# efeslab/Atom

Hardware: AMD Instinct MI355X
Metric: effective TOPS, W4A4 group-128 GEMM + 128 INT8 outlier cols, fp16 out (higher is better)
Workload: dtype int4xint4 exact integer dot (BF6-coded on the f8f6f4 MFMA; INT8 MFMA for the keeper), fp32 dequant, fp16 out

## Files before the change

atom_amd/csrc/gemm_w4a4_f6.hip:

```cpp
#include <type_traits>
#include "common.h"
#include "quant_math.h"

namespace atom {

__global__ void splitk_reduce_kernel(const float *ws, half_t *D, int64_t MN, int splits);

namespace f6 {

typedef const __attribute__((address_space(1))) void *gptr_t;
typedef __attribute__((address_space(3))) void *lptr_t;
typedef int v8i __attribute__((ext_vector_type(8)));
typedef float v16f __attribute__((ext_vector_type(16)));

constexpr int TN = 2;
constexpr int PITCH = 104;
constexpr float kMagic = 12582912.0f;
constexpr int kMagicBits = 0x4B400000;

template <int BM_, int BN_, int TM_, int NS_, int OCC_ = 2, int FS_ = 0>
struct Cfg {
  static constexpr int FS = FS_;
  static constexpr int FS32 = FS_ == 1;
  static constexpr int OCC = OCC_;
// ... 1068 lines not shown
    auto dmak1 = [&](int i) { if (i == 0) issue_keeper<C>(p, 1, slot_of(G + 1), wave, lane, m0, n0); };
    auto tr_sel = [&]() {
      if constexpr ((ABL & 16) != 0) {
        if (tr_on) tr_i += 6;
        tr_on = blockIdx.x == 0 && tr_i + 6 <= 78 && (s < 3 || s == G / 2 || s == G / 2 + 1 || s + 3 >= G);
      }
    };
    kstamp(3);
    if constexpr ((ABL & 1024) != 0) {
      auto dma4f = [&](int i) { if (i < C::GLDS) issue_int4_piece<C>(p, s + 2, lds + 2 * C::STAGE_BYTES, wave, lane, m0, n0, i); };
      for (; s + 2 < G; ++s) p_step<C, false, ABL>(R, lds, lds + C::STAGE_BYTES, wm, wn, lane, c, sync, dma4f, stamp);
    }
    for (; s + 2 < G; ++s) { tr_sel(); p_step<C, false, ABL>(R, slot_of(s), slot_of(s + 1), wm, wn, lane, c, sync, dma4, stamp); }
    if (G >= 2) { tr_sel(); p_step<C, false, ABL>(R, slot_of(s), slot_of(s + 1), wm, wn, lane, c, sync, dmak0, stamp); ++s; }
    tr_sel();
    p_step<C, true, ABL>(R, slot_of(s), slot_of(s + 1), wm, wn, lane, c, sync, dmak1, stamp);
  }
  kstamp(4);
  p_drain<C>(R, c);
  kstamp(5);
  asm volatile("s_waitcnt vmcnt(0)" ::: "memory");
  __builtin_amdgcn_s_barrier();
  kstamp(6);
  if constexpr (!(ABL & 128)) p_keeper<C>(slot_of(G), slot_of(G + 1), wm, wn, lane, c);
  kstamp(7);

#pragma unroll
  for (int tb = 0; tb < 8; ++tb) {
    const int m = m0 + wm * 128 + p_row(tb) + 2 * l15;
    if (m >= p.M) continue;
#pragma unroll
    for (int h = 0; h < 2; ++h) {
      const int n = n0 + wn * 64 + 32 * h + 8 * kb;
      if (n >= p.N) continue;
      v4u o;
      half_t *ov = reinterpret_cast<half_t *>(&o);
#pragma unroll
      for (int r = 0; r < 4; ++r) {
        ov[2 * r] = f2h(c[2 * h][tb][r]);
        ov[2 * r + 1] = f2h(c[2 * h + 1][tb][r]);
      }
      if constexpr ((ABL & 64) != 0) { if (o.x != 0x12345678u) continue; }
      *reinterpret_cast<v4u *>(p.D + (int64_t)m * p.N + n) = o;
    }
  }
  if constexpr ((ABL & 16) != 0) {
    kstamp(8);
    asm volatile("s_waitcnt vmcnt(0)" ::: "memory");
    kstamp(9);
    if (blockIdx.x == 0) {
      if (lane == 0) trl[79] = (unsigned)__builtin_amdgcn_s_memrealtime();
      asm volatile("s_waitcnt lgkmcnt(0)" ::: "memory");
      for (int i = lane; i < 80; i += 64) reinterpret_cast<unsigned *>(p.Dsz)[wave * 80 + i] = trl[i];
    }
  }
}

template <class C>
struct QC {
  static constexpr int SB_OFF = C::SB_OFF;
  static constexpr int STAGE = C::SB_OFF + C::BN * 4;
  static constexpr int LDS_BYTES = 3 * STAGE;
  static_assert(LDS_BYTES <= 160 * 1024 && STAGE + (32 * 3 + 1) * PITCH + 100 < 65536, "q kernel: stage layout / ds offsets");
};

typedef float v2f_t __attribute__((ext_vector_type(2)));
#ifdef ATOM_SA_B32
struct QSa {
  float v;
  __device__ __forceinline__ QSa() = default;
  __device__ __forceinline__ QSa(float f) : v(f) {}
  __device__ __forceinline__ operator float() const { return v; }
};
#else
struct QSa {
  v2f_t p;
  __device__ __forceinline__ QSa() = default;
  __device__ __forceinline__ QSa(float f) : p{0.f, f} {}
  __device__ __forceinline__ QSa(v2f_t q) : p(q) {}
  __device__ __forceinline__ operator float() const { asm volatile("" ::"v"(p)); return p.y; }
};
#endif

template <class C, bool PAIR = false>
struct QRegs {
  v8i af[4];
  v8i bf[3];
  float sb[2][PAIR ? 4 : 8];
  QSa sa[4];
  v4f_t acc[2][2];
  int aW[2][3], aA[2][3], aS[2], aB[2];
#ifdef ATOM_F6_PAIR128
  int aWp[2][3];
#endif
};

template <int SL> __device__ __forceinline__ constexpr int q_set() { return SL == 2 ? 1 : 0; }
template <class C, int SL> __device__ __forceinline__ constexpr int q_imm() { return SL == 1 ? QC<C>::STAGE : 0; }

template <class C, int SL>
__device__ __forceinline__ v8i q_frag(const char *lds, const int (&a)[2][3], int off, int ro) {
  const char *b = lds + (SL < 0 ? ro : q_imm<C, SL>()) + off;
  const v2u x = *reinterpret_cast<const v2u *>(b + a[q_set<SL>()][0]);
  const v2u y = *reinterpret_cast<const v2u *>(b + a[q_set<SL>()][1]);
  const v2u z = *reinterpret_cast<const v2u *>(b + a[q_set<SL>()][2]);
  asm volatile("" ::: "memory");
  return v8i{(int)x.x, (int)x.y, (int)y.x, (int)y.y, (int)z.x, (int)z.y, 0, 0};
}
#ifdef ATOM_F6_PAIR128
template <class C, int SL>
__device__ __forceinline__ void q_frag_pair(const char *lds, const int (&a)[2][3], int off, int ro, v8i &f0, v8i &f1) {
  const char *b = lds + (SL < 0 ? ro : q_imm<C, SL>()) + off;
  const v4u x = *reinterpret_cast<const v4u *>(b + a[q_set<SL>()][0]);
  const v4u y = *reinterpret_cast<const v4u *>(b + a[q_set<SL>()][1]);
  const v4u z = *reinterpret_cast<const v4u *>(b + a[q_set<SL>()][2]);
  asm volatile("" ::: "memory");
  f0 = v8i{(int)x.x, (int)x.y, (int)y.x, (int)y.y, (int)z.x, (int)z.y, 0, 0};
  f1 = v8i{(int)x.z, (int)x.w, (int)y.z, (int)y.w, (int)z.z, (int)z.w, 0, 0};
}
#endif
template <class C, int SL, class RG>
__device__ __forceinline__ QSa q_scale(const char *lds, const RG &R, int off, int ro) {
#ifdef ATOM_SA_B32
  return *reinterpret_cast<const float *>(lds + (SL < 0 ? ro : q_imm<C, SL>()) + off + R.aS[q_set<SL>()] + 4);
#else
  return QSa(*reinterpret_cast<const v2f_t *>(lds + (SL < 0 ? ro : q_imm<C, SL>()) + off + R.aS[q_set<SL>()]));
#endif
}
template <class C, int SL, class RG>
__device__ __forceinline__ void q_load_sb(const char *lds, RG &R, int h, int ro) {
  const char *b = lds + (SL < 0 ? ro : q_imm<C, SL>()) + QC<C>::SB_OFF + 128 * h + R.aB[q_set<SL>()];
  if constexpr (sizeof(R.sb[0]) == 4 * sizeof(float)) {
    const float *f = reinterpret_cast<const float *>(b);
#pragma unroll
    for (int k = 0; k < 4; ++k) R.sb[h][k] = f[2 * k];
  } else {
    const v4f_t lo = *reinterpret_cast<const v4f_t *>(b), hi = *reinterpret_cast<const v4f_t *>(b + 16);
#pragma unroll
    for (int k = 0; k < 4; ++k) { R.sb[h][k] = lo[k]; R.sb[h][4 + k] = hi[k]; }
  }
}

__device__ __forceinline__ void q_dma16x3(unsigned m0v, unsigned voff, const void *sbase) {
  asm volatile("s_mov_b32 m0, %0\n\ts_nop 0\n\tglobal_load_lds_dwordx4 %1, %2\n\tglobal_load_lds_dwordx4 %1, %2 offset:1024\n\t"
               "global_load_lds_dwordx4 %1, %2 offset:2048" ::"s"(m0v), "v"(voff), "s"(sbase) : "memory");
}
__device__ __forceinline__ void q_dma16(unsigned m0v, unsigned voff, const void *sbase) {
  asm volatile("s_mov_b32 m0, %0\n\ts_nop 0\n\tglobal_load_lds_dwordx4 %1, %2" ::"s"(m0v), "v"(voff), "s"(sbase) : "memory");
}
struct QDma {
  unsigned voffW, voffA, voffX;
  int m0W, m0A, m0X;
  int xkind;
};
template <class C, int DS>
__device__ __forceinline__ void q_piece(const QDma &d, const uint8_t *wsrc, const uint8_t *asrc, const float *sbsrc, int i) {
  constexpr int base = DS * QC<C>::STAGE;
  if (i == 0) q_dma16x3(base + d.m0W, d.voffW, wsrc);
  else if (i == 3) q_dma16x3(base + d.m0A, d.voffA, asrc);
  else if (i == 6) {
    const void *xb = d.xkind == 1 ? (const void *)wsrc : (d.xkind == 2 ? (const void *)asrc : (const void *)sbsrc);
    q_dma16(base + d.m0X, d.voffX, xb);
  }
}

struct QNoEarly { __device__ __forceinline__ void operator()(int) const {} };
template <class C, int SL, bool PAIR, class FS, class FD, class FE = QNoEarly>
__device__ __forceinline__ void q_step(QRegs<C, PAIR> &R, const char *lds, float (&c)[4][8][4], FS sync, FD mid, int ro = 0, int rn = 0,
                                       bool LAST = false, FE early = FE(), unsigned *tp = nullptr) {
  constexpr int NX = SL < 0 ? -1 : (SL + 1) % 3;
  auto stamp = [&](int k) {
    if (tp) { __builtin_amdgcn_sched_barrier(0); const unsigned t_ = (unsigned)__builtin_amdgcn_s_memtime(); if ((threadIdx.x & 63) == 0) tp[k] = t_; __builtin_amdgcn_sched_barrier(0); }
  };
#pragma unroll
  for (int i = 0; i < 16; ++i) {
    const int tb = p_tb(i), h = p_h(i);
    __builtin_amdgcn_sched_barrier(0);
    stamp(i);
    if (i == 8) { stamp(16); sync(); stamp(17); }
    __builtin_amdgcn_sched_barrier(0);
#pragma unroll
    for (int k = 0; k < 2; ++k)
      R.acc[i & 1][k] = __builtin_amdgcn_mfma_scale_f32_16x16x128_f8f6f4(R.af[2 * h + k], R.bf[p_buf(tb)], v4f_t{0.f, 0.f, 0.f, 0.f}, 3, 3, 0, 0, 0, 0);
    __builtin_amdgcn_sched_barrier(0);
    stamp(32 + 2 * i);
    if (h == 1 && i < 12 && tb + 2 < 8) {
      R.bf[p_buf(tb + 2)] = q_frag<C, SL>(lds, R.aA, p_row(tb + 2) * PITCH, ro);
      R.sa[(tb + 2) & 3] = q_scale<C, SL>(lds, R, p_row(tb + 2) * PITCH, ro);
    }
    if (!LAST) {
      if (i == 12) {
        R.bf[2] = q_frag<C, NX>(lds, R.aA, p_row(0) * PITCH, rn);
        R.sa[0] = q_scale<C, NX>(lds, R, p_row(0) * PITCH, rn);
      }
      if (i == 13) {
#ifdef ATOM_F6_PAIR128
        q_frag_pair<C, NX>(lds, R.aWp, p_row(0) * PITCH, rn, R.af[0], R.af[1]);
#else
        R.af[0] = q_frag<C, NX>(lds, R.aW, p_row(0) * PITCH, rn);
        R.af[1] = q_frag<C, NX>(lds, R.aW, p_row(1) * PITCH, rn);
#endif
      }
      if (i == 15) {
#ifdef ATOM_F6_PAIR128
        q_frag_pair<C, NX>(lds, R.aWp, p_row(2) * PITCH, rn, R.af[2], R.af[3]);
#else
        R.af[2] = q_frag<C, NX>(lds, R.aW, p_row(2) * PITCH, rn);
        R.af[3] = q_frag<C, NX>(lds, R.aW, p_row(3) * PITCH, rn);
#endif
        R.bf[1] = q_frag<C, NX>(lds, R.aA, p_row(1) * PITCH, rn);
        R.sa[1] = q_scale<C, NX>(lds, R, p_row(1) * PITCH, rn);
      }
    }
    if (i >= 8) mid(i - 8);
    else early(i);
    if (tp) asm volatile("s_waitcnt lgkmcnt(0)" ::: "memory");
    stamp(33 + 2 * i);
    __builtin_amdgcn_sched_barrier(0);
    {
      const int j = (i + 15) & 15, dtb = p_tb(j), dh = p_h(j);
      deq_pair<PAIR>(R.acc[j & 1][0], R.acc[j & 1][1], R.sa[dtb & 3], R.sb[dh], c[2 * dh][dtb], c[2 * dh + 1][dtb]);
    }
    __builtin_amdgcn_sched_barrier(0);
    if (!LAST && i == 14) q_load_sb<C, NX>(lds, R, 0, rn);
    if (i == 0) q_load_sb<C, SL>(lds, R, 1, ro);
  }
  stamp(18);
}

template <class C, bool STORE, int NTB>
__device__ __forceinline__ void q_keeper(const GemmParams &p, const char *slot, const char *slot1, int wm, int wn, int lane, float (&c)[4][NTB][4],
                                         int m0, int n0) {
  constexpr bool MERGED = true;
  const int l15 = lane & 15, kb = lane >> 4;
  const int sw = (l15 >> 1) & 3;
  const char *pw = slot + (wn * 64 + 2 * l15) * 64 + ((kb ^ sw) << 4);
  const char *pa = slot + (C::BN + wm * (16 * NTB) + 2 * l15) * 64 + ((kb ^ sw) << 4);
  const char *psa = slot + C::KP_SA_OFF + (wm * (16 * NTB) + 2 * l15) * 4;
  const char *psb = slot + C::SB_OFF + (wn * 64 + 8 * kb) * 2;
  v4i af[4], bf[2];
  v4i af1[4], bf1[2];
  const long d1 = slot1 - slot;
  float sb[2][8], sa[2];
  v4i acc[2][2];
  const v4i magic = {kMagicBits, kMagicBits, kMagicBits, kMagicBits};
#pragma unroll
  for (int fb = 0; fb < 4; ++fb) af[fb] = __builtin_bit_cast(v4i, *reinterpret_cast<const v4u *>(pw + p_row(fb) * 64));
  bf[0] = __builtin_bit_cast(v4i, *reinterpret_cast<const v4u *>(pa + p_row(0) * 64));
  bf[1] = __builtin_bit_cast(v4i, *reinterpret_cast<const v4u *>(pa + p_row(1) * 64));
  if constexpr (MERGED) {
#pragma unroll
    for (int fb = 0; fb < 4; ++fb) af1[fb] = __builtin_bit_cast(v4i, *reinterpret_cast<const v4u *>(pw + d1 + p_row(fb) * 64));
    bf1[0] = __builtin_bit_cast(v4i, *reinterpret_cast<const v4u *>(pa + d1 + p_row(0) * 64));
    bf1[1] = __builtin_bit_cast(v4i, *reinterpret_cast<const v4u *>(pa + d1 + p_row(1) * 64));
  }
  half_t sah[2];
  sah[0] = *reinterpret_cast<const half_t *>(psa + p_row(0) * 4);
  sah[1] = *reinterpret_cast<const half_t *>(psa + p_row(1) * 4);
#pragma unroll
  for (int h = 0; h < 2; ++h) {
    const v4u w = *reinterpret_cast<const v4u *>(psb + 64 * h);
    const half_t *hv = reinterpret_cast<const half_t *>(&w);
#pragma unroll
    for (int j = 0; j < 8; ++j) { sb[h][j] = (float)hv[j]; asm volatile("" : "+v"(sb[h][j])); }
  }
  auto store_block = [&](int tb) {
    const int m = m0 + wm * (16 * NTB) + p_row(tb) + 2 * l15;
    if (m >= p.M) return;
#pragma unroll
    for (int h = 0; h < 2; ++h) {
      const int n = n0 + wn * 64 + 32 * h + 8 * kb;
      if (n >= p.N) continue;
      v4u o;
      half_t *ov = reinterpret_cast<half_t *>(&o);
#pragma unroll
      for (int r = 0; r < 4; ++r) {
        ov[2 * r] = f2h(c[2 * h][tb][r]);
        ov[2 * r + 1] = f2h(c[2 * h + 1][tb][r]);
      }
      *reinterpret_cast<v4u *>(p.D + (int64_t)m * p.N + n) = o;
    }
  };
  auto dequant = [&](int j) {
    const int tb = j >> 1, h = j & 1;
    v4f_t f[2];
#pragma unroll
    for (int k = 0; k < 2; ++k)
#pragma unroll
      for (int r = 0; r < 4; ++r) f[k][r] = __int_as_float(acc[j & 1][k][r]) - kMagic;
    deq_pair<false>(f[0], f[1], sa[tb & 1], sb[h], c[2 * h][tb], c[2 * h + 1][tb]);
  };
#pragma unroll
  for (int i = 0; i < 2 * NTB; ++i) {
    const int tb = i >> 1, h = i & 1;
    __builtin_amdgcn_sched_barrier(0);
    if (h == 0) sa[tb & 1] = (float)sah[tb & 1];
#pragma unroll
    for (int k = 0; k < 2; ++k) acc[i & 1][k] = __builtin_amdgcn_mfma_i32_16x16x64_i8(af[2 * h + k], bf[tb & 1], magic, 0, 0, 0);
    if constexpr (MERGED) {
#pragma unroll
      for (int k = 0; k < 2; ++k) acc[i & 1][k] = __builtin_amdgcn_mfma_i32_16x16x64_i8(af1[2 * h + k], bf1[tb & 1], acc[i & 1][k], 0, 0, 0);
    }
    __builtin_amdgcn_sched_barrier(0);
    if (h == 1 && tb + 2 < NTB) {
      bf[tb & 1] = __builtin_bit_cast(v4i, *reinterpret_cast<const v4u *>(pa + p_row(tb + 2) * 64));
      if constexpr (MERGED) bf1[tb & 1] = __builtin_bit_cast(v4i, *reinterpret_cast<const v4u *>(pa + d1 + p_row(tb + 2) * 64));
      sah[tb & 1] = *reinterpret_cast<const half_t *>(psa + p_row(tb + 2) * 4);
    }
    if constexpr (STORE) { if (h == 1 && tb >= 1) store_block(tb - 1); }
    __builtin_amdgcn_sched_barrier(0);
    if (i > 0) dequant(i - 1);
  }
  __builtin_amdgcn_sched_barrier(0);
  dequant(2 * NTB - 1);
  if constexpr (STORE) store_block(NTB - 1);
}

template <class C, int GU = 0, bool TR = false, bool PAIR = false>
__global__ __launch_bounds__(C::NT, C::OCC) void gemm_w4a4_f6q_kernel(GemmParams p) {
  extern __shared__ __attribute__((aligned(16))) char lds[];
  static_assert(C::BM == 256 && C::BN == 256 && C::WM == 128 && C::NS == 3 && C::NW == 8, "q kernel: 256x256, 8 waves of 64 x 128");
  using Q = QC<C>;
  unsigned *trb = nullptr;
  auto kstamp = [&](int k) {
    if constexpr (TR) {
      if (trb) { const unsigned t = (unsigned)__builtin_amdgcn_s_memtime(); if ((threadIdx.x & 63) == 0) trb[k] = t; }
    }
  };
  if constexpr (TR) {
    if (blockIdx.x == 0 || blockIdx.x == gridDim.x - 1) {
      trb = reinterpret_cast<unsigned *>(p.Dsz) + ((blockIdx.x ? 8 : 0) + (threadIdx.x >> 6)) * 128;
      if ((threadIdx.x & 63) == 0) trb[62] = (unsigned)__builtin_amdgcn_s_memrealtime();
    }
    kstamp(0);
  }
  const int tid = threadIdx.x;
  const int lane = tid & 63;
  const int wave = __builtin_amdgcn_readfirstlane(tid >> 6);
  __builtin_assume(wave >= 0 && wave < C::NW);
  const int wm = wave / C::WGN, wn = wave % C::WGN;
  const int nbn = (p.N + C::BN - 1) / C::BN, nbm = (p.M + C::BM - 1) / C::BM;
  const int nwg = nbm * nbn;
  int id = blockIdx.x;
  {
    const int q = nwg >> 3, r = nwg & 7, xcd = id & 7, k = id >> 3;
    id = (xcd < r ? xcd * (q + 1) : r * (q + 1) + (xcd - r) * q) + k;
  }
  constexpr int GM = 4;
  const int band = id / (GM * nbn), inband = id % (GM * nbn);
  const int rows_in_band = min(GM, nbm - band * GM);
  const int bm = band * GM + inband % rows_in_band, bn = inband / rows_in_band;
  const int m0 = bm * C::BM, n0 = bn * C::BN;

  float c[4][8][4];
#pragma unroll
  for (int a = 0; a < 4; ++a)
#pragma unroll
    for (int b = 0; b < 8; ++b)
#pragma unroll
      for (int r = 0; r < 4; ++r) c[a][b][r] = 0.f;

  const int G = p.G;
  QDma d;
  d.voffW = d.voffA = (unsigned)(wave * 3072 + lane * 16);
  d.m0W = wave * 3072;
  d.m0A = C::A_OFF + wave * 3072;
  d.xkind = wave < 2 ? 1 : (wave < 4 ? 2 : 3);
  d.voffX = (unsigned)((wave < 4 ? (24 + (wave & 1)) * 1024 : 0) + lane * 16);
  d.m0X = wave < 2 ? (24 + wave) * 1024 : (wave < 4 ? C::A_OFF + (24 + (wave & 1)) * 1024 : Q::SB_OFF);
  const int64_t wstep = p.f6_rows_b * PITCH, astep = p.f6_rows_a * PITCH;
  const uint8_t *wsrc0 = p.B4 + (int64_t)n0 * PITCH, *asrc0 = p.A4 + (int64_t)m0 * PITCH;
  const float *sbsrc0 = p.sB32 + n0;
  auto slot_of = [&](int stage) { return lds + (stage % 3) * Q::STAGE; };
  auto issue_all = [&](auto ds, int g) {
    constexpr int DS = decltype(ds)::value;
#pragma unroll
    for (int i = 0; i < 7; ++i) q_piece<C, DS>(d, wsrc0 + g * wstep, asrc0 + g * astep, sbsrc0 + (int64_t)g * p.f6_rows_b, i);
  };
  const bool early1 = G >= 6;
  issue_all(std::integral_constant<int, 0>(), 0);
  if (!early1) {
    if (G >= 2) issue_all(std::integral_constant<int, 1>(), 1);
    else issue_keeper<C>(p, 0, slot_of(1), wave, lane, m0, n0);
  }
  kstamp(1);
  asm volatile("s_waitcnt vmcnt(0)" ::: "memory");
  __builtin_amdgcn_s_barrier();
  kstamp(2);

  const int l15 = lane & 15, kb = lane >> 4;
  QRegs<C, PAIR> R;
  {
    const int lw = wn * 64 * PITCH + l15 * (2 * PITCH) + kb * 24;
    const int la = C::A_OFF + wm * 128 * PITCH + l15 * (2 * PITCH);
#pragma unroll
    for (int st = 0; st < 2; ++st) {
#pragma unroll
      for (int k = 0; k < 3; ++k) {
        R.aW[st][k] = lw + 8 * k + st * 2 * Q::STAGE;
        R.aA[st][k] = la + kb * 24 + 8 * k + st * 2 * Q::STAGE;
        asm volatile("" : "+v"(R.aW[st][k]), "+v"(R.aA[st][k]));
#ifdef ATOM_F6_PAIR128
        R.aWp[st][k] = ((wn * 64 * PITCH + l15 * (2 * PITCH) + kb * 48 + 16 * k + st * 2 * Q::STAGE) & ~15);
        asm volatile("" : "+v"(R.aWp[st][k]));
#endif
      }
      R.aS[st] = la + 96 + st * 2 * Q::STAGE;
      R.aB[st] = (wn * 64 + 8 * kb) * 4 + st * 2 * Q::STAGE;
      asm volatile("" : "+v"(R.aS[st]), "+v"(R.aB[st]));
    }
    R.bf[2] = q_frag<C, 0>(lds, R.aA, p_row(0) * PITCH, 0);
#pragma unroll
    for (int fb = 0; fb < 4; ++fb) R.af[fb] = q_frag<C, 0>(lds, R.aW, p_row(fb) * PITCH, 0);
    R.bf[1] = q_frag<C, 0>(lds, R.aA, p_row(1) * PITCH, 0);
    R.bf[0] = R.bf[1];
    R.sa[0] = q_scale<C, 0>(lds, R, p_row(0) * PITCH, 0);
    R.sa[1] = q_scale<C, 0>(lds, R, p_row(1) * PITCH, 0);
    R.sa[2] = 0.f;
    R.sa[3] = 0.f;
    q_load_sb<C, 0>(lds, R, 0, 0);
    q_load_sb<C, 0>(lds, R, 1, 0);
#pragma unroll
    for (int k = 0; k < 2; ++k) R.acc[1][k] = v4f_t{0.f, 0.f, 0.f, 0.f};
  }
  if constexpr (TR) { asm volatile("s_waitcnt lgkmcnt(0)" ::: "memory"); kstamp(3); }
  auto sync = [&]() {
    asm volatile("s_waitcnt vmcnt(0)" ::: "memory");
    __builtin_amdgcn_s_barrier();
  };
  auto reg = [&](auto sl, int s) {
    constexpr int SL = decltype(sl)::value;
    if constexpr (TR) { if (s < 44) kstamp(16 + s); }
    const int g = s + 2;
    const uint8_t *wsrc = wsrc0 + g * wstep, *asrc = asrc0 + g * astep;
    const float *sbsrc = sbsrc0 + (int64_t)g * p.f6_rows_b;
    unsigned *tp = nullptr;
    if constexpr (TR) { if (trb && s == 9) tp = trb + 64; }
    q_step<C, SL, PAIR>(R, lds, c, sync, [&](int i) { q_piece<C, (SL + 2) % 3>(d, wsrc, asrc, sbsrc, i); }, 0, 0, false, QNoEarly(), tp);
  };
  using S0 = std::integral_constant<int, 0>;
  using S1 = std::integral_constant<int, 1>;
  using S2 = std::integral_constant<int, 2>;
  int s = 0;
  if (early1) {
    if constexpr (TR) kstamp(16);
    const uint8_t *wsrc = wsrc0 + 2 * wstep, *asrc = asrc0 + 2 * astep;
    const float *sbsrc = sbsrc0 + (int64_t)2 * p.f6_rows_b;
    q_step<C, 0, PAIR>(R, lds, c, sync, [&](int i) { q_piece<C, 2>(d, wsrc, asrc, sbsrc, i); }, 0, 0, false,
                 [&](int i) { q_piece<C, 1>(d, wsrc0 + wstep, asrc0 + astep, sbsrc0 + p.f6_rows_b, i); });
    reg(S1(), 1);
    reg(S2(), 2);
    s = 3;
  }
  for (; s + 4 < G; s += 3) { reg(S0(), s); reg(S1(), s + 1); reg(S2(), s + 2); }
  if (s + 2 < G) { reg(S0(), s); ++s; }
  if (s + 2 < G) { reg(S1(), s); ++s; }
  for (; s < G; ++s) {
    if constexpr (TR) { if (s < 44) kstamp(16 + s); }
    const int g = s + 2;
    const int dsl = g % 3;
    const uint8_t *wsrc = wsrc0 + g * wstep, *asrc = asrc0 + g * astep;
    const float *sbsrc = sbsrc0 + (int64_t)g * p.f6_rows_b;
    q_step<C, -1, PAIR>(R, lds, c, sync,
                  [&](int i) {
                    if (g < G) {
                      if (dsl == 0) q_piece<C, 0>(d, wsrc, asrc, sbsrc, i);
                      else if (dsl == 1) q_piece<C, 1>(d, wsrc, asrc, sbsrc, i);
                      else q_piece<C, 2>(d, wsrc, asrc, sbsrc, i);
                    } else if (i == 0) issue_keeper<C>(p, g - G, slot_of(g), wave, lane, m0, n0);
                  },
                  (s % 3) * Q::STAGE, ((s + 1) % 3) * Q::STAGE, s + 1 == G);
  }
  deq_pair<PAIR>(R.acc[1][0], R.acc[1][1], R.sa[3], R.sb[1], c[2][7], c[3][7]);
  kstamp(4);
  asm volatile("s_waitcnt vmcnt(0)" ::: "memory");
  __builtin_amdgcn_s_barrier();
  kstamp(5); kstamp(6);
  q_keeper<C, GU == 0>(p, slot_of(G), slot_of(G + 1), wm, wn, lane, c, m0, n0);
  if constexpr (TR) {
    kstamp(7);
    asm volatile("s_waitcnt vmcnt(0)" ::: "memory");
    kstamp(8);
    if (trb && (threadIdx.x & 63) == 0) trb[63] = (unsigned)__builtin_amdgcn_s_memrealtime();
  }
  if constexpr (GU == 0) return;

  if constexpr (GU != 0) {
    constexpr bool SIM = GU == 1;
    float *am = reinterpret_cast<float *>(lds + ((G + 2) % 3) * Q::STAGE);
#pragma unroll
    for (int tb = 0; tb < 8; ++tb) {
      float mx = 0.f;
#pragma unroll
      for (int k = 0; k < 2; ++k)
#pragma unroll
        for (int r = 0; r < 4; ++r) {
          const float h = silu_mul<SIM>((float)f2h(c[k][tb][r]), (float)f2h(c[2 + k][tb][r]));
          c[k][tb][r] = h;
          mx = fmaxf(mx, fabsf(h));
        }
      mx = fmaxf(mx, __shfl_xor(mx, 16));
      mx = fmaxf(mx, __shfl_xor(mx, 32));
      if (kb == 0) am[wave * 128 + p_row(tb) + 2 * l15] = mx;
    }
    __syncthreads();
    const bool keeper_blk = bn == nbn - 1;
    const GateUpOut &o = p.gu;
    const int N_inter = p.N >> 1;
#pragma unroll
    for (int tb = 0; tb < 8; ++tb) {
      const int t = p_row(tb) + 2 * l15;
      const float *ap = am + wm * 4 * 128 + t;
      const float amax = fmaxf(fmaxf(ap[0], ap[128]), fmaxf(ap[256], ap[384]));
      const GroupScale gs = group_scale<SIM>(amax, keeper_blk, o.clip);
      float tr[8];
#pragma unroll
      for (int k = 0; k < 2; ++k)
#pragma unroll
        for (int r = 0; r < 4; ++r) tr[2 * r + k] = group_code<SIM>(c[k][tb][r], gs);
      const int64_t m = m0 + wm * 128 + t;
      if (m >= p.M) continue;
      const half_t sh = f2h(gs.s_store);
      if (keeper_blk) {
        *reinterpret_cast<v2u *>(o.o8 + m * kKeeper + wn * 32 + kb * 8) = pack_codes8(tr, true);
      } else {
        const v6u_t f = bf6_fields(tr);
        uint8_t *dst = o.o6 + ((int64_t)bn * o.o6_rows + m) * PITCH;
        uint8_t *d6 = dst + wn * 24 + kb * 6;
        if ((kb & 1) == 0) {
          *reinterpret_cast<unsigned *>(d6) = f[0];
          *reinterpret_cast<unsigned short *>(d6 + 4) = (unsigned short)f[1];
        } else {
          *reinterpret_cast<unsigned short *>(d6) = (unsigned short)f[0];
          *reinterpret_cast<unsigned *>(d6 + 2) = (f[0] >> 16) | (f[1] << 16);
        }
        if (wn == 0 && kb == 0) *reinterpret_cast<v2u *>(dst + 96) = f6_scale_words(__builtin_bit_cast(unsigned short, sh));
      }
      if (wn == 0 && kb == 0) store_token_scale(keeper_blk ? o.s8 : (o.s4 + (int64_t)bn * o.ld4), m, sh, o.ref_layout);
      if (o.xq) {
        v4u q;
        half_t *qv = reinterpret_cast<half_t *>(&q);
#pragma unroll
        for (int j = 0; j < 8; ++j) qv[j] = dequant_half(tr[j], gs);
        *reinterpret_cast<v4u *>(o.xq + m * N_inter + bn * 128 + wn * 32 + kb * 8) = q;
      }
    }
    return;
  }
}

template <class C, int GU = 0, bool TR = false, bool PAIR = false>
static int launch_q(const GemmParams &p, hipStream_t s) {
  static std::atomic<uint64_t> attr_done{0};
  if (ensure_max_lds(reinterpret_cast<const void *>(&gemm_w4a4_f6q_kernel<C, GU, TR, PAIR>), QC<C>::LDS_BYTES, attr_done) != ATOM_OK) return ATOM_ERR_LAUNCH;
  const int nbm = (p.M + C::BM - 1) / C::BM, nbn = (p.N + C::BN - 1) / C::BN;
  hipLaunchKernelGGL((gemm_w4a4_f6q_kernel<C, GU, TR, PAIR>), dim3((unsigned)(nbm * nbn)), dim3(C::NT), QC<C>::LDS_BYTES, s, p);
  return check_launch();
}

struct QkDma {
  unsigned voff, voffX;
// ... 444 lines not shown
  asm volatile("s_waitcnt vmcnt(0)" ::: "memory");
  __builtin_amdgcn_s_barrier();
  q_keeper<C, true>(p, slot_of(G), slot_of(G + 1), wm, wn, lane, c, m0, n0);
}

template <class C>
static int launch_q2(const GemmParams &p, hipStream_t s) {
  static std::atomic<uint64_t> attr_done{0};
  constexpr int LDS = 3 * QC<C>::STAGE;
  if (ensure_max_lds(reinterpret_cast<const void *>(&gemm_w4a4_f6q2_kernel<C>), LDS, attr_done) != ATOM_OK) return ATOM_ERR_LAUNCH;
  const int nbm = (p.M + C::BM - 1) / C::BM, nbn = (p.N + C::BN - 1) / C::BN;
  hipLaunchKernelGGL((gemm_w4a4_f6q2_kernel<C>), dim3((unsigned)(nbm * nbn)), dim3(C::NT), LDS, s, p);
  return check_launch();
}

template <class C, int ABL = 0>
static int launch_p(const GemmParams &p, hipStream_t s) {
  constexpr int lds_bytes = C::LDS_BYTES + ((ABL & 16) ? 8 * 80 * 4 : 0);
  static_assert(lds_bytes <= 160 * 1024, "LDS");
  static std::atomic<uint64_t> attr_done{0};
  if (ensure_max_lds(reinterpret_cast<const void *>(&gemm_w4a4_f6p_kernel<C, ABL>), lds_bytes, attr_done) != ATOM_OK) return ATOM_ERR_LAUNCH;
  const int nbm = (p.M + C::BM - 1) / C::BM, nbn = (p.N + C::BN - 1) / C::BN;
  hipLaunchKernelGGL((gemm_w4a4_f6p_kernel<C, ABL>), dim3((unsigned)(nbm * nbn)), dim3(C::NT), lds_bytes, s, p);
  return check_launch();
}

template <class C, bool SK = false, int KG = 1, bool PH = false, bool TR = false>
static int launch_x16(const GemmParams &p, hipStream_t s) {
  static std::atomic<uint64_t> attr_done{0};
  constexpr int XCH = KG == 4 ? C::NW * 4 * (16 * 80 + 8 * 4 * 64 * 4) : C::NW * KG * (C::WM / 2) * (144 + 64 * 4);
  constexpr int LDS = (KG > 1 ? (KG * C::NS * C::STAGE_BYTES > XCH ? KG * C::NS * C::STAGE_BYTES : XCH) : C::LDS_BYTES) + (TR ? 2048 : 0);
  static_assert(LDS <= 160 * 1024, "LDS");
  if (ensure_max_lds(reinterpret_cast<const void *>(&gemm_w4a4_f6x16_kernel<C, SK, KG, PH, TR>), LDS, attr_done) != ATOM_OK) return ATOM_ERR_LAUNCH;
  const int nbm = (p.M + C::BM - 1) / C::BM, nbn = (p.N + C::BN - 1) / C::BN;
  hipLaunchKernelGGL((gemm_w4a4_f6x16_kernel<C, SK, KG, PH, TR>), dim3((unsigned)(nbm * nbn), (unsigned)(SK ? p.splits : 1)), dim3(C::NT * KG),
                     LDS, s, p);
  if (SK) {
    const int64_t MN = (int64_t)p.M * p.N;
    hipLaunchKernelGGL(splitk_reduce_kernel, dim3((unsigned)((MN / 8 + 255) / 256)), dim3(256), 0, s, p.ws, p.D, MN, p.splits);
  }
  return check_launch();
}

template <class C, bool SK, int ABL = 0>
static int launch(const GemmParams &p, hipStream_t s) {
  static std::atomic<uint64_t> attr_done{0};
  if (ensure_max_lds(reinterpret_cast<const void *>(&gemm_w4a4_f6_kernel<C, SK, ABL>), C::LDS_BYTES, attr_done) != ATOM_OK) return ATOM_ERR_LAUNCH;
  const int nbm = (p.M + C::BM - 1) / C::BM, nbn = (p.N + C::BN - 1) / C::BN;
  hipLaunchKernelGGL((gemm_w4a4_f6_kernel<C, SK, ABL>), dim3((unsigned)(nbm * nbn), (unsigned)(SK ? p.splits : 1)), dim3(C::NT),
                     C::LDS_BYTES, s, p);
  if (SK) {
    const int64_t MN = (int64_t)p.M * p.N;
    hipLaunchKernelGGL(splitk_reduce_kernel, dim3((unsigned)((MN / 8 + 255) / 256)), dim3(256), 0, s, p.ws, p.D, MN, p.splits);
  }
  return check_launch();
}

}

int launch_gemm_f6_gateup(const GemmParams &p, int sim, hipStream_t s) {
  using C = f6::Cfg<256, 256, 4, 3>;
  if (p.b_pairs) return sim ? f6::launch_q<C, 1, false, true>(p, s) : f6::launch_q<C, 2, false, true>(p, s);
  return sim ? f6::launch_q<C, 1>(p, s) : f6::launch_q<C, 2>(p, s);
}

static bool f6_128_f32_scales(const GemmParams &p) {
  const int64_t t128 = (int64_t)((p.M + 127) / 128) * ((p.N + 127) / 128);
  return p.sB32 && (t128 + 511) / 512 <= (t128 + 767) / 768;
}

#ifdef ATOM_TOOLS
static bool launch_gemm_f6_tools(const GemmParams &p, int cfg, hipStream_t s, int &st) {
  using C256 = f6::Cfg<256, 256, 4, 3>;
  const bool split = p.splits > 1 && p.ws;
  st = ATOM_ERR_INVALID_ARG;
  if (cfg == 116 || cfg == 1016 || cfg == 1005 || cfg == 1009 || cfg == 2016 || cfg == 2017) {
    GemmParams q = p;
    q.Dsz = trace_ptr();
    if (!q.Dsz || (!p.sB32 && cfg != 116 && cfg != 1016)) return true;
    st = cfg == 116    ? f6::launch<C256, false, 16>(q, s)
         : cfg == 1016 ? f6::launch_p<C256, 16>(q, s)
         : cfg == 1005 ? f6::launch_x16<f6::Cfg<128, 128, 2, 2, 3, 1>, false, 2, false, true>(q, s)
         : cfg == 1009 ? f6::launch_x16<f6::Cfg<64, 128, 1, 3, 3, 1>, false, 2, false, true>(q, s)
         : cfg == 2016 ? f6::launch_q<C256, 0, true>(q, s)
                       : f6::launch_qk<f6::Cfg<128, 128, 2, 3, 3, 1>, true>(q, s);
    return true;
  }
#define ATOM_CASE(c, call) case c: st = call(p, s); return true;
#define ATOM_CASE2(c, cond, a, b) case c: st = (cond) ? a(p, s) : b(p, s); return true;
#define ATOM_ABL(a) ATOM_CASE(100 + a, (f6::launch<C256, false, a>))
#define ATOM_ABLP(a) ATOM_CASE(1000 + a, (f6::launch_p<C256, a>))
#define ATOM_ABLQ(a) case 2100 + a: if (p.sB32) st = f6::launch_qk<f6::Cfg<128, 128, 2, 3, 3, 1>, false, a>(p, s); return true;
  switch (cfg) {
    ATOM_ABL(1) ATOM_ABL(2) ATOM_ABL(3) ATOM_ABL(4) ATOM_ABL(6) ATOM_ABL(7) ATOM_ABL(8) ATOM_ABL(10) ATOM_ABL(14) ATOM_ABL(15) ATOM_ABL(32)
    ATOM_ABLQ(0) ATOM_ABLQ(1) ATOM_ABLQ(2) ATOM_ABLQ(4) ATOM_ABLQ(8) ATOM_ABLQ(16) ATOM_ABLQ(17) ATOM_ABLQ(6) ATOM_ABLQ(14) ATOM_ABLQ(15) ATOM_ABLQ(31)
    ATOM_ABLQ(3) ATOM_ABLQ(5) ATOM_ABLQ(9) ATOM_ABLQ(7) ATOM_ABLQ(11) ATOM_ABLQ(13)
    ATOM_ABLP(1) ATOM_ABLP(2) ATOM_ABLP(3) ATOM_ABLP(4) ATOM_ABLP(6) ATOM_ABLP(7) ATOM_ABLP(8) ATOM_ABLP(10) ATOM_ABLP(14) ATOM_ABLP(15)
    ATOM_ABLP(64) ATOM_ABLP(128) ATOM_ABLP(192) ATOM_ABLP(207) ATOM_ABLP(256) ATOM_ABLP(257) ATOM_ABLP(512) ATOM_ABLP(513) ATOM_ABLP(768) ATOM_ABLP(769)
    ATOM_ABLP(520) ATOM_ABLP(9) ATOM_ABLP(1024) ATOM_ABLP(2048) ATOM_ABLP(4096)
    ATOM_CASE2(F6_64x128, split, (f6::launch<f6::Cfg<64, 128, 2, 3>, true>), (f6::launch<f6::Cfg<64, 128, 2, 3>, false>))
    ATOM_CASE(F6_256x256_32, (f6::launch<C256, false>))
    ATOM_CASE(F6_256x128_P, (f6::launch<f6::Cfg<256, 128, 4, 2>, false>))
    ATOM_CASE(F6_128x128_32, (f6::launch<f6::Cfg<128, 128, 2, 2, 3>, false>))
    case F6_128x128:
      if (!split) return false;
      st = f6_128_f32_scales(p) ? f6::launch_x16<f6::Cfg<128, 128, 2, 2, 3, 1>, true>(p, s) : f6::launch_x16<f6::Cfg<128, 128, 2, 2, 3, 2>, true>(p, s);
      return true;
    ATOM_CASE2(F6_128x128_KG2_S2, p.sB32, (f6::launch_x16<f6::Cfg<128, 128, 2, 2, 3, 1>, false, 2>), (f6::launch_x16<f6::Cfg<128, 128, 2, 2, 3, 2>, false, 2>))
    ATOM_CASE2(F6_64x128_KG2, p.sB32, (f6::launch_x16<f6::Cfg<64, 128, 1, 3, 3, 1>, false, 2, true>), (f6::launch_x16<f6::Cfg<64, 128, 1, 3, 3, 2>, false, 2, true>))
    ATOM_CASE2(F6_64x128_KG4, p.sB32, (f6::launch_x16<f6::Cfg<64, 128, 1, 2, 4, 1>, false, 4>), (f6::launch_x16<f6::Cfg<64, 128, 1, 2, 4, 2>, false, 4>))
    case 51: if (!p.sB32) return false;
      st = f6::launch_x16<f6::Cfg<128, 128, 2, 2, 3, 1>>(p, s); return true;
    ATOM_CASE(52, (f6::launch_x16<f6::Cfg<128, 128, 2, 2, 3, 2>>))
    ATOM_CASE(53, (f6::launch_x16<f6::Cfg<128, 128, 2, 2, 3>>))
    ATOM_CASE(40, (f6::launch_x16<C256>))
    case 41: case 42: if (!p.sB32) return false;
      st = cfg == 41 ? f6::launch_x16<f6::Cfg<256, 256, 4, 3, 2, 1>>(p, s) : f6::launch_x16<f6::Cfg<256, 256, 2, 3, 4, 1>>(p, s);
      return true;
    ATOM_CASE2(F6_128x128_8W, split, (f6::launch_x16<f6::Cfg<128, 128, 1, 2, 3>, true>), (f6::launch_x16<f6::Cfg<128, 128, 1, 2, 3>>))
    ATOM_CASE(F6_256x256_P, (f6::launch_p<C256>))
  }
#undef ATOM_CASE
#undef ATOM_CASE2
#undef ATOM_ABL
#undef ATOM_ABLP
#undef ATOM_ABLQ
  return false;
}
#endif

int launch_gemm_f6(const GemmParams &p, int cfg, hipStream_t s) {
#ifdef ATOM_TOOLS
  int st;
  if (launch_gemm_f6_tools(p, cfg, s, st)) return st;
#endif
  if (cfg == F6_MID) {
    const int r = launch_gemm_f6_mid(p, s);
    if (r != ATOM_ERR_SHAPE) return r;
    cfg = F6_128x128;
  }
  if (cfg == F6_256x128) {
    if (p.sB32 && p.G >= 2) return f6::launch_q2<f6::Cfg<256, 128, 2, 3, 2, 1>>(p, s);
    cfg = F6_128x128;
  }
  if (cfg == F6_128x128)
    return f6_128_f32_scales(p) ? f6::launch_x16<f6::Cfg<128, 128, 2, 2, 3, 1>>(p, s) : f6::launch_x16<f6::Cfg<128, 128, 2, 2, 3, 2>>(p, s);
  if (cfg == F6_128x128_KG2) {
    if (p.sB32 && p.G >= 7 && ATOM_TUNE("ATOM_QK", 1)) return f6::launch_qk<f6::Cfg<128, 128, 2, 3, 3, 1>>(p, s);
    if (p.sB32) return f6::launch_x16<f6::Cfg<128, 128, 2, 3, 3, 1>, false, 2>(p, s);
    return f6::launch_x16<f6::Cfg<128, 128, 2, 3, 3, 2>, false, 2>(p, s);
  }
  if (!p.sB32) return f6::launch_p<f6::Cfg<256, 256, 4, 3>>(p, s);
  if (p.b_pairs) return f6::launch_q<f6::Cfg<256, 256, 4, 3>, 0, false, true>(p, s);
  return f6::launch_q<f6::Cfg<256, 256, 4, 3>>(p, s);
}

}
```

Baseline: 2792.

## Pair activation-scale LDS loads, use immediate-offset LDS addressing, unguarded full-tile stores

Adds an SA2 mode for the paired-B, non-split kernel that loads two rows' activation scales per LDS access into a v2f register and precomputes per-slot scale addresses, so the main loop issues fewer scale reads. Fragment loads switch to address-space-3 pointers with a constant immediate offset, trimming per-load VALU address arithmetic. The keeper epilogue gains a WHOLE path that drops the M/N bounds checks and uses one precomputed byte offset for interior tiles. In exchange the kernel holds a 3x4 table of scale addresses in registers, which may raise VGPR pressure, and it now carries an extra epilogue instantiation.

```diff
diff --git a/atom_amd/csrc/gemm_w4a4_f6.hip b/atom_amd/csrc/gemm_w4a4_f6.hip
--- a/atom_amd/csrc/gemm_w4a4_f6.hip
+++ b/atom_amd/csrc/gemm_w4a4_f6.hip
@@ -1174,14 +1174,20 @@
 };
 #endif
 
-template <class C, bool PAIR = false>
+template <class C, bool PAIR = false, bool SA2 = false>
 struct QRegs {
   v8i af[4];
   v8i bf[3];
   float sb[2][PAIR ? 4 : 8];
   QSa sa[4];
+  v2f_t sa2[2];
   v4f_t acc[2][2];
   int aW[2][3], aA[2][3], aS[2], aB[2];
+  int aS2[3][4];
+  __device__ __forceinline__ float tscale(int tb) const {
+    if constexpr (SA2) return sa2[(tb & 3) >> 1][tb & 1];
+    else return sa[tb & 3];
+  }
 #ifdef ATOM_F6_PAIR128
   int aWp[2][3];
 #endif
@@ -1190,12 +1196,30 @@
 template <int SL> __device__ __forceinline__ constexpr int q_set() { return SL == 2 ? 1 : 0; }
 template <class C, int SL> __device__ __forceinline__ constexpr int q_imm() { return SL == 1 ? QC<C>::STAGE : 0; }
 
-template <class C, int SL>
+template <class T>
+__device__ __forceinline__ T q_ld0(int a, int imm) {
+#if defined(__HIP_DEVICE_COMPILE__)
+  typedef const __attribute__((address_space(3))) char *cp_t;
+  typedef const __attribute__((address_space(3))) T *tp_t;
+  return *(tp_t)((cp_t)(unsigned)a + imm);
+#else
+  return T{};
+#endif
+}
+template <class C, int SL, bool Z = false>
 __device__ __forceinline__ v8i q_frag(const char *lds, const int (&a)[2][3], int off, int ro) {
   const char *b = lds + (SL < 0 ? ro : q_imm<C, SL>()) + off;
-  const v2u x = *reinterpret_cast<const v2u *>(b + a[q_set<SL>()][0]);
-  const v2u y = *reinterpret_cast<const v2u *>(b + a[q_set<SL>()][1]);
-  const v2u z = *reinterpret_cast<const v2u *>(b + a[q_set<SL>()][2]);
+  v2u x, y, z;
+  if constexpr (Z) {
+    const int imm = (SL < 0 ? 0 : q_imm<C, SL>()) + off, r = SL < 0 ? ro : 0;
+    x = q_ld0<v2u>(a[q_set<SL>()][0] + r, imm);
+    y = q_ld0<v2u>(a[q_set<SL>()][1] + r, imm);
+    z = q_ld0<v2u>(a[q_set<SL>()][2] + r, imm);
+  } else {
+    x = *reinterpret_cast<const v2u *>(b + a[q_set<SL>()][0]);
+    y = *reinterpret_cast<const v2u *>(b + a[q_set<SL>()][1]);
+    z = *reinterpret_cast<const v2u *>(b + a[q_set<SL>()][2]);
+  }
   asm volatile("" ::: "memory");
   return v8i{(int)x.x, (int)x.y, (int)y.x, (int)y.y, (int)z.x, (int)z.y, 0, 0};
 }
@@ -1218,6 +1242,11 @@
 #else
   return QSa(*reinterpret_cast<const v2f_t *>(lds + (SL < 0 ? ro : q_imm<C, SL>()) + off + R.aS[q_set<SL>()]));
 #endif
+}
+template <class C, int SL, class RG>
+__device__ __forceinline__ v2f_t q_scale2(const char *lds, const RG &R, int j, int ro) {
+  const int a = R.aS2[SL < 0 ? 0 : SL][j] + (SL < 0 ? ro : 0);
+  return v2f_t{q_ld0<float>(a, 100), q_ld0<float>(a, PITCH + 100)};
 }
 template <class C, int SL, class RG>
 __device__ __forceinline__ void q_load_sb(const char *lds, RG &R, int h, int ro) {
@@ -1257,8 +1286,8 @@
 }
 
 struct QNoEarly { __device__ __forceinline__ void operator()(int) const {} };
-template <class C, int SL, bool PAIR, class FS, class FD, class FE = QNoEarly>
-__device__ __forceinline__ void q_step(QRegs<C, PAIR> &R, const char *lds, float (&c)[4][8][4], FS sync, FD mid, int ro = 0, int rn = 0,
+template <class C, int SL, bool PAIR, bool SA2, class FS, class FD, class FE = QNoEarly>
+__device__ __forceinline__ void q_step(QRegs<C, PAIR, SA2> &R, const char *lds, float (&c)[4][8][4], FS sync, FD mid, int ro = 0, int rn = 0,
                                        bool LAST = false, FE early = FE(), unsigned *tp = nullptr) {
   constexpr int NX = SL < 0 ? -1 : (SL + 1) % 3;
   auto stamp = [&](int k) {
@@ -1277,32 +1306,35 @@
     __builtin_amdgcn_sched_barrier(0);
     stamp(32 + 2 * i);
     if (h == 1 && i < 12 && tb + 2 < 8) {
-      R.bf[p_buf(tb + 2)] = q_frag<C, SL>(lds, R.aA, p_row(tb + 2) * PITCH, ro);
-      R.sa[(tb + 2) & 3] = q_scale<C, SL>(lds, R, p_row(tb + 2) * PITCH, ro);
+      R.bf[p_buf(tb + 2)] = q_frag<C, SL, SA2>(lds, R.aA, p_row(tb + 2) * PITCH, ro);
+      if constexpr (SA2) {
+        if ((tb & 1) == 0) R.sa2[((tb + 2) & 3) >> 1] = q_scale2<C, SL>(lds, R, (tb + 2) >> 1, ro);
+      } else R.sa[(tb + 2) & 3] = q_scale<C, SL>(lds, R, p_row(tb + 2) * PITCH, ro);
     }
     if (!LAST) {
       if (i == 12) {
-        R.bf[2] = q_frag<C, NX>(lds, R.aA, p_row(0) * PITCH, rn);
-        R.sa[0] = q_scale<C, NX>(lds, R, p_row(0) * PITCH, rn);
+        R.bf[2] = q_frag<C, NX, SA2>(lds, R.aA, p_row(0) * PITCH, rn);
+        if constexpr (!SA2) R.sa[0] = q_scale<C, NX>(lds, R, p_row(0) * PITCH, rn);
       }
       if (i == 13) {
 #ifdef ATOM_F6_PAIR128
         q_frag_pair<C, NX>(lds, R.aWp, p_row(0) * PITCH, rn, R.af[0], R.af[1]);
 #else
-        R.af[0] = q_frag<C, NX>(lds, R.aW, p_row(0) * PITCH, rn);
-        R.af[1] = q_frag<C, NX>(lds, R.aW, p_row(1) * PITCH, rn);
+        R.af[0] = q_frag<C, NX, SA2>(lds, R.aW, p_row(0) * PITCH, rn);
+        R.af[1] = q_frag<C, NX, SA2>(lds, R.aW, p_row(1) * PITCH, rn);
 #endif
       }
       if (i == 15) {
 #ifdef ATOM_F6_PAIR128
         q_frag_pair<C, NX>(lds, R.aWp, p_row(2) * PITCH, rn, R.af[2], R.af[3]);
 #else
-        R.af[2] = q_frag<C, NX>(lds, R.aW, p_row(2) * PITCH, rn);
-        R.af[3] = q_frag<C, NX>(lds, R.aW, p_row(3) * PITCH, rn);
+        R.af[2] = q_frag<C, NX, SA2>(lds, R.aW, p_row(2) * PITCH, rn);
+        R.af[3] = q_frag<C, NX, SA2>(lds, R.aW, p_row(3) * PITCH, rn);
 #endif
-        R.bf[1] = q_frag<C, NX>(lds, R.aA, p_row(1) * PITCH, rn);
-        R.sa[1] = q_scale<C, NX>(lds, R, p_row(1) * PITCH, rn);
-      }
+        R.bf[1] = q_frag<C, NX, SA2>(lds, R.aA, p_row(1) * PITCH, rn);
+        if constexpr (!SA2) R.sa[1] = q_scale<C, NX>(lds, R, p_row(1) * PITCH, rn);
+      }
+      if constexpr (SA2) { if (i == 14) R.sa2[0] = q_scale2<C, NX>(lds, R, 0, rn); }
     }
     if (i >= 8) mid(i - 8);
     else early(i);
@@ -1311,7 +1343,7 @@
     __builtin_amdgcn_sched_barrier(0);
     {
       const int j = (i + 15) & 15, dtb = p_tb(j), dh = p_h(j);
-      deq_pair<PAIR>(R.acc[j & 1][0], R.acc[j & 1][1], R.sa[dtb & 3], R.sb[dh], c[2 * dh][dtb], c[2 * dh + 1][dtb]);
+      deq_pair<PAIR>(R.acc[j & 1][0], R.acc[j & 1][1], R.tscale(dtb), R.sb[dh], c[2 * dh][dtb], c[2 * dh + 1][dtb]);
     }
     __builtin_amdgcn_sched_barrier(0);
     if (!LAST && i == 14) q_load_sb<C, NX>(lds, R, 0, rn);
@@ -1320,7 +1352,7 @@
   stamp(18);
 }
 
-template <class C, bool STORE, int NTB>
+template <class C, bool STORE, int NTB, bool WHOLE = false>
 __device__ __forceinline__ void q_keeper(const GemmParams &p, const char *slot, const char *slot1, int wm, int wn, int lane, float (&c)[4][NTB][4],
                                          int m0, int n0) {
   constexpr bool MERGED = true;
@@ -1356,13 +1388,18 @@
 #pragma unroll
     for (int j = 0; j < 8; ++j) { sb[h][j] = (float)hv[j]; asm volatile("" : "+v"(sb[h][j])); }
   }
+  unsigned dvoff = 0;
+  if constexpr (STORE && WHOLE) {
+    dvoff = (unsigned)(((wm * (16 * NTB) + 2 * l15) * p.N + wn * 64 + 8 * kb) * 2);
+    asm volatile("" : "+v"(dvoff));
+  }
   auto store_block = [&](int tb) {
     const int m = m0 + wm * (16 * NTB) + p_row(tb) + 2 * l15;
-    if (m >= p.M) return;
+    if constexpr (!WHOLE) { if (m >= p.M) return; }
 #pragma unroll
     for (int h = 0; h < 2; ++h) {
       const int n = n0 + wn * 64 + 32 * h + 8 * kb;
-      if (n >= p.N) continue;
+      if constexpr (!WHOLE) { if (n >= p.N) continue; }
       v4u o;
       half_t *ov = reinterpret_cast<half_t *>(&o);
 #pragma unroll
@@ -1370,7 +1407,12 @@
         ov[2 * r] = f2h(c[2 * h][tb][r]);
         ov[2 * r + 1] = f2h(c[2 * h + 1][tb][r]);
       }
-      *reinterpret_cast<v4u *>(p.D + (int64_t)m * p.N + n) = o;
+      if constexpr (WHOLE) {
+        char *dtb = reinterpret_cast<char *>(p.D + ((int64_t)(m0 + p_row(tb)) * p.N + n0));
+        *reinterpret_cast<v4u *>(dtb + dvoff + 64 * h) = o;
+      } else {
+        *reinterpret_cast<v4u *>(p.D + (int64_t)m * p.N + n) = o;
+      }
     }
   };
   auto dequant = [&](int j) {
@@ -1481,7 +1523,12 @@
   kstamp(2);
 
   const int l15 = lane & 15, kb = lane >> 4;
-  QRegs<C, PAIR> R;
+#ifdef ATOM_Q_NO_SA2
+  constexpr bool SA2 = false;
+#else
+  constexpr bool SA2 = PAIR && GU == 0;
+#endif
+  QRegs<C, PAIR, SA2> R;
   {
     const int lw = wn * 64 * PITCH + l15 * (2 * PITCH) + kb * 24;
     const int la = C::A_OFF + wm * 128 * PITCH + l15 * (2 * PITCH);
@@ -1499,17 +1546,32 @@
       }
       R.aS[st] = la + 96 + st * 2 * Q::STAGE;
       R.aB[st] = (wn * 64 + 8 * kb) * 4 + st * 2 * Q::STAGE;
-      asm volatile("" : "+v"(R.aS[st]), "+v"(R.aB[st]));
-    }
-    R.bf[2] = q_frag<C, 0>(lds, R.aA, p_row(0) * PITCH, 0);
-#pragma unroll
-    for (int fb = 0; fb < 4; ++fb) R.af[fb] = q_frag<C, 0>(lds, R.aW, p_row(fb) * PITCH, 0);
-    R.bf[1] = q_frag<C, 0>(lds, R.aA, p_row(1) * PITCH, 0);
+      if constexpr (!SA2) asm volatile("" : "+v"(R.aS[st]));
+      asm volatile("" : "+v"(R.aB[st]));
+    }
+    if constexpr (SA2) {
+#pragma unroll
+      for (int sl = 0; sl < 3; ++sl)
+#pragma unroll
+        for (int j = 0; j < 4; ++j) {
+          R.aS2[sl][j] = la + sl * Q::STAGE + p_row(2 * j) * PITCH;
+          asm volatile("" : "+v"(R.aS2[sl][j]));
+        }
+    }
+    R.bf[2] = q_frag<C, 0, SA2>(lds, R.aA, p_row(0) * PITCH, 0);
+#pragma unroll
+    for (int fb = 0; fb < 4; ++fb) R.af[fb] = q_frag<C, 0, SA2>(lds, R.aW, p_row(fb) * PITCH, 0);
+    R.bf[1] = q_frag<C, 0, SA2>(lds, R.aA, p_row(1) * PITCH, 0);
     R.bf[0] = R.bf[1];
-    R.sa[0] = q_scale<C, 0>(lds, R, p_row(0) * PITCH, 0);
-    R.sa[1] = q_scale<C, 0>(lds, R, p_row(1) * PITCH, 0);
-    R.sa[2] = 0.f;
-    R.sa[3] = 0.f;
+    if constexpr (SA2) {
+      R.sa2[0] = q_scale2<C, 0>(lds, R, 0, 0);
+      R.sa2[1] = v2f_t{0.f, 0.f};
+    } else {
+      R.sa[0] = q_scale<C, 0>(lds, R, p_row(0) * PITCH, 0);
+      R.sa[1] = q_scale<C, 0>(lds, R, p_row(1) * PITCH, 0);
+      R.sa[2] = 0.f;
+      R.sa[3] = 0.f;
+    }
     q_load_sb<C, 0>(lds, R, 0, 0);
     q_load_sb<C, 0>(lds, R, 1, 0);
 #pragma unroll
@@ -1522,12 +1584,16 @@
   };
   auto reg = [&](auto sl, int s) {
     constexpr int SL = decltype(sl)::value;
+#ifndef ATOM_TR_LOOP_ONLY
     if constexpr (TR) { if (s < 44) kstamp(16 + s); }
+#endif
     const int g = s + 2;
     const uint8_t *wsrc = wsrc0 + g * wstep, *asrc = asrc0 + g * astep;
     const float *sbsrc = sbsrc0 + (int64_t)g * p.f6_rows_b;
     unsigned *tp = nullptr;
+#ifndef ATOM_TR_LOOP_ONLY
     if constexpr (TR) { if (trb && s == 9) tp = trb + 64; }
+#endif
     q_step<C, SL, PAIR>(R, lds, c, sync, [&](int i) { q_piece<C, (SL + 2) % 3>(d, wsrc, asrc, sbsrc, i); }, 0, 0, false, QNoEarly(), tp);
   };
   using S0 = std::integral_constant<int, 0>;
@@ -1548,7 +1614,9 @@
   if (s + 2 < G) { reg(S0(), s); ++s; }
   if (s + 2 < G) { reg(S1(), s); ++s; }
   for (; s < G; ++s) {
+#ifndef ATOM_TR_LOOP_ONLY
     if constexpr (TR) { if (s < 44) kstamp(16 + s); }
+#endif
     const int g = s + 2;
     const int dsl = g % 3;
     const uint8_t *wsrc = wsrc0 + g * wstep, *asrc = asrc0 + g * astep;
@@ -1563,12 +1631,22 @@
                   },
                   (s % 3) * Q::STAGE, ((s + 1) % 3) * Q::STAGE, s + 1 == G);
   }
-  deq_pair<PAIR>(R.acc[1][0], R.acc[1][1], R.sa[3], R.sb[1], c[2][7], c[3][7]);
+  deq_pair<PAIR>(R.acc[1][0], R.acc[1][1], R.tscale(7), R.sb[1], c[2][7], c[3][7]);
   kstamp(4);
   asm volatile("s_waitcnt vmcnt(0)" ::: "memory");
   __builtin_amdgcn_s_barrier();
   kstamp(5); kstamp(6);
-  q_keeper<C, GU == 0>(p, slot_of(G), slot_of(G + 1), wm, wn, lane, c, m0, n0);
+  if constexpr (GU == 0) {
+#ifdef ATOM_Q_NO_WHOLE
+    const bool whole = false;
+#else
+    const bool whole = m0 + C::BM <= p.M && n0 + C::BN <= p.N && p.N <= (1 << 21);
+#endif
+    if (whole) q_keeper<C, true, 8, true>(p, slot_of(G), slot_of(G + 1), wm, wn, lane, c, m0, n0);
+    else q_keeper<C, true, 8, false>(p, slot_of(G), slot_of(G + 1), wm, wn, lane, c, m0, n0);
+  } else {
+    q_keeper<C, false>(p, slot_of(G), slot_of(G + 1), wm, wn, lane, c, m0, n0);
+  }
   if constexpr (TR) {
     kstamp(7);
     asm volatile("s_waitcnt vmcnt(0)" ::: "memory");
@@ -2179,7 +2257,7 @@
          : cfg == 1016 ? f6::launch_p<C256, 16>(q, s)
          : cfg == 1005 ? f6::launch_x16<f6::Cfg<128, 128, 2, 2, 3, 1>, false, 2, false, true>(q, s)
          : cfg == 1009 ? f6::launch_x16<f6::Cfg<64, 128, 1, 3, 3, 1>, false, 2, false, true>(q, s)
-         : cfg == 2016 ? f6::launch_q<C256, 0, true>(q, s)
+         : cfg == 2016 ? (q.b_pairs ? f6::launch_q<C256, 0, true, true>(q, s) : f6::launch_q<C256, 0, true>(q, s))
                        : f6::launch_qk<f6::Cfg<128, 128, 2, 3, 3, 1>, true>(q, s);
     return true;
   }
```

New measurement: 2832 (median of 6 runs). 1.01x the previous value.
